# magnate3/dpdk_dc_sand

Measured on AMD Instinct MI355X. Metric: int8 voltage Gsamples/s ingested + beams/s, 64-ant 4096-ch; % HBM roofline, higher is better.
Workload: dtype int8

## Files before the change

### dpdk_dc_sand_amd/csrc/bf_fused.hpp

```cpp
#pragma once

#include <type_traits>

#include "bf_fused_plan.hpp"
#include "bf_mfma.hpp"
#include "bf_phase.hpp"

namespace bf {

typedef uint32_t u32x4_t __attribute__((ext_vector_type(4)));
typedef uint32_t u32x2_t __attribute__((ext_vector_type(2)));

struct FusedArgs {
  const uint8_t* raw;
  const float4* dv;
  const float* gain;
  const uint32_t* table;
  size_t table_bytes;
  void* y;
  int delay_channels, B, C, T, A, M, S, NT, nslabs, xcd_order;
  int path, order;
  int c_count;
  long long base_ch;
  double ctot, ts, k, t0, batch_dt;
  float out_scale;
  int ch_run;
};

__device__ __forceinline__ void apply_gain(float g, float* re, float* im) {
  *re = __fmul_rn(*re, g);
  *im = __fmul_rn(*im, g);
}


constexpr uint32_t kSelP0 = 0x05040100u;
constexpr uint32_t kSelP1 = 0x07060302u;
typedef int i32x4_t __attribute__((ext_vector_type(4)));

__device__ __forceinline__ i32x4_t mfma_i8(i32x4_t a, i32x4_t b, i32x4_t c) {
  return __builtin_amdgcn_mfma_i32_16x16x64_i8(a, b, c, 0, 0, 0);
}

__device__ __forceinline__ int coef8_byte(int k, int cl, int nts, int limb) {
  const int s = k >> 6, h = (k >> 4) & 3, j = k & 15, tau = cl >> 4, row = cl & 15;
  return ((((s * nts + tau) * 2 + limb) * 64) + row + 16 * h) * 16 + j;
}

template <bool Pow2 = false>
__device__ __forceinline__ uint32_t requant_bits(int y, float s) {
  constexpr float kMagic = 12582912.0f;
  float v;
  if constexpr (Pow2) {
    v = __builtin_fmaf(static_cast<float>(y), s, kMagic);
  } else {
#pragma clang fp contract(off)
    v = static_cast<float>(y) * s + kMagic;
  }
  return __float_as_uint(__builtin_amdgcn_fmed3f(v, kMagic - 127.0f, kMagic + 127.0f));
}

__device__ __forceinline__ uint32_t pack_low_bytes(uint32_t a, uint32_t b, uint32_t c, uint32_t d) {
  const uint32_t ab = __builtin_amdgcn_perm(b, a, 0x0c0c0400u);
  const uint32_t cd = __builtin_amdgcn_perm(d, c, 0x0c0c0400u);
  return __builtin_amdgcn_perm(cd, ab, 0x05040100u);
}

__device__ __forceinline__ void transpose_rows4(uint32_t (&v)[4]) {
  auto a = __builtin_amdgcn_permlane32_swap(v[0], v[2], false, false);
  auto b = __builtin_amdgcn_permlane32_swap(v[1], v[3], false, false);
  auto c = __builtin_amdgcn_permlane16_swap(a[0], b[0], false, false);
  auto d = __builtin_amdgcn_permlane16_swap(a[1], b[1], false, false);
  v[0] = c[0];
  v[1] = c[1];
  v[2] = d[0];
  v[3] = d[1];
}

__device__ __forceinline__ void lds_barrier() {
  __atomic_signal_fence(__ATOMIC_SEQ_CST);
  __builtin_amdgcn_s_waitcnt(0xc07f);
  __builtin_amdgcn_s_barrier();
  __atomic_signal_fence(__ATOMIC_SEQ_CST);
}

constexpr int kLayoutNatural = 0, kLayoutW32 = 1, kLayoutW32H = 2;
int launch_q14_table(const FusedArgs& P, uint32_t* out, int layout, hipStream_t st);

using FusedKernel = void (*)(FusedArgs);

template <class F>
FusedKernel with_bools(F f) {
  return f();
}
template <class F, class... Bs>
FusedKernel with_bools(F f, bool b, Bs... bs) {
  return b ? with_bools([&](auto... cs) -> FusedKernel { return f(std::true_type{}, cs...); }, bs...)
           : with_bools([&](auto... cs) -> FusedKernel { return f(std::false_type{}, cs...); }, bs...);
}

int launch_planned(FusedKernel k, const FusedPlan& p, FusedArgs P, hipStream_t st);
int launch_wide(const FusedPlan& p, FusedArgs P, hipStream_t st);
int launch_w32(const FusedPlan& p, FusedArgs P, hipStream_t st);

}
```

### dpdk_dc_sand_amd/csrc/bf_fused_dims.hpp

```cpp
#pragma once

#include <cstddef>
#include <cstdint>
#include <cstring>

#ifdef __HIPCC__
#define BF_HD __host__ __device__
#else
#define BF_HD
#endif

namespace bf {

constexpr size_t kMaxLds = 160 * 1024;

inline size_t coef_lds_bytes(int S, int nts) { return static_cast<size_t>(S) * nts * 2 * 64 * 16; }

constexpr int kGroup = 4;

constexpr int kF32StageRow = 36;
constexpr size_t kF32StageBytes = 4 * 64 * kF32StageRow * 4;

constexpr int kWideGroup = 2;
BF_HD inline int wide_padded_steps(int A) {
  return 2 * kWideGroup * ((((A + 15) >> 4) + 2 * kWideGroup - 1) / (2 * kWideGroup));
}
constexpr int kWidePSteps = 16;

constexpr int kW32Beams = 32;
constexpr int kW32TChannels = 4;
constexpr int kW32RChannels = 8;
BF_HD inline int w32_table_steps(int A) { return 4 * ((((A + 31) >> 5) + 3) / 4); }
BF_HD inline bool w32_table_fits(int A) { return w32_table_steps(A) <= 8; }
inline size_t w32_table_bytes(int B, int C, int A, int M) {
  return static_cast<size_t>(B) * C * ((M + 31) / 32) * 1024 * w32_table_steps(A) * 4;
}
BF_HD inline size_t w32_lds_bytes(int A) {
  return static_cast<size_t>(w32_table_steps(A)) * 4 * 2 * 64 * 16 + 4 * 64 * 4;
}

inline bool scale_is_pow2(float s) {
  uint32_t u;
  memcpy(&u, &s, 4);
  const uint32_t e = (u >> 23) & 255;
  return (u & 0x7fffffu) == 0 && e > 0 && e < 255;
}

}
```

### dpdk_dc_sand_amd/csrc/bf_fused_plan.cpp

```cpp
#include "bf_fused_plan.hpp"

#include <algorithm>
#include <cstdarg>
#include <cstdio>

namespace bf {
namespace {

FusedPlan refuse(const char* fmt, ...) __attribute__((format(printf, 1, 2)));
FusedPlan refuse(const char* fmt, ...) {
  FusedPlan p{};
  p.status = BF_ERR_ARG;
  va_list ap;
  va_start(ap, fmt);
  vsnprintf(p.error, sizeof(p.error), fmt, ap);
  va_end(ap);
  return p;
}

FusedPlan with_grid(FusedPlan p, long long grid, const char* too_large = "grid too large") {
  if (grid >= (1LL << 31)) return refuse("bf_beamform_fused: %s", too_large);
  p.grid = static_cast<unsigned>(grid);
  return p;
}

struct Shape : FusedShape {
  explicit Shape(const FusedShape& s) : FusedShape(s) {}
  int path() const { return flags & BF_FUSED_PATH_MASK; }
  int order() const { return flags & BF_FUSED_ORDER_MASK; }
  int S() const { return (2 * A + 31) / 32; }
  int S8() const { return (2 * A + 63) / 64; }
  int NT() const { return (2 * M + 15) / 16; }
  long long items() const { return static_cast<long long>(B) * C; }
  bool small() const { return A <= 64 && T <= 256; }
  bool offsets31() const { return static_cast<unsigned long long>(A) * C * T * 4 < (1ull << 31); }
  bool lane_offsets32(int rows) const {
    return static_cast<size_t>(rows) * C * T * 4 + static_cast<size_t>(T) * 4 < (1ull << 32);
  }
  bool slab_xcd_order(int nslabs) const { return nslabs > 1 && order() != BF_FUSED_ORDER_CHANNEL; }
  long long slab_grid(long long columns, int nslabs, bool xcd) const {
    return xcd ? (columns + 7) / 8 * 8 * nslabs : columns * nslabs;
  }
  bool item_xcd_order() const {
    if (order() == BF_FUSED_ORDER_CHANNEL) return false;
    if (order() == BF_FUSED_ORDER_XCD) return (C & 7) == 0;
    return (C & 7) == 0 && M >= 8;
  }
  bool wide_fits() const {
    return A >= 16 && lane_offsets32(12) && coef_lds_bytes(wide_padded_steps(A), 1) <= kMaxLds;
  }
  bool wide_p2_fits() const {
    return A == 256 && T == 256 && M % 32 == 0 && delay_channels == 1 && !gains && offsets31();
  }
  bool i8_w32_fits() const { return A >= 32 && (T & 1) == 0 && lane_offsets32(24) && w32_lds_bytes(A) <= kMaxLds; }
  bool w32r_fits() const {
    return w32_table_steps(A) == 8 && A > 224 && T == 256 && M % kW32Beams == 0 && offsets31() &&
           static_cast<unsigned long long>(B) * 2 * C * T * 2 * M < (1ull << 31);
  }
};

void item_slabs(const Shape& s, FusedPlan& p) {
  p.nts = s.NT() >= 2 ? 2 : 1;
  p.full = p.nts == 2 ? (2 * s.M) % 32 == 0 : 2 * s.M == 16;
  p.nslabs = (s.NT() + p.nts - 1) / p.nts;
  p.xcd_order = s.item_xcd_order();
}

FusedPlan plan_item(const Shape& s, FusedPlan p) {
  p.family = FusedFamily::Item;
  item_slabs(s, p);
  p.staged = !p.i8out && s.M == 16;
  p.pow2 = p.i8out && scale_is_pow2(s.out_scale);
  p.lds = coef_lds_bytes(s.S(), p.nts) + (p.staged ? kF32StageBytes : 0);
  return with_grid(p, p.nslabs * s.items(), "too many (batch, channel) items");
}

FusedPlan plan_generic(const Shape& s, FusedPlan p) {
  p.family = FusedFamily::Generic;
  p.nts = s.NT() >= 2 && coef_lds_bytes(s.S(), 2) <= kMaxLds ? 2 : 1;
  p.nslabs = (s.NT() + p.nts - 1) / p.nts;
  p.lds = coef_lds_bytes(s.S(), p.nts);
  if (p.lds > kMaxLds) return refuse("bf_beamform_fused: n_ants=%d too large", s.A);
  p.xcd_order = s.slab_xcd_order(p.nslabs);
  return with_grid(p, s.slab_grid(s.items(), p.nslabs, p.xcd_order));
}

FusedPlan plan_wide(const Shape& s, FusedPlan p) {
  if (!p.exact && s.wide_p2_fits() && s.order() != BF_FUSED_ORDER_CHANNEL) {
    p.family = FusedFamily::WideP2;
    p.nts = 2;
    p.nslabs = s.M / 32;
    const long long units = static_cast<long long>(s.B) * p.nslabs;
    const int cus = std::max(1, s.cus);
    p.ch_run = static_cast<int>(std::min<long long>(s.C, std::max<long long>(1, (s.C * units + cus - 1) / cus)));
    const long long groups = static_cast<long long>(s.B) * ((s.C + p.ch_run - 1) / p.ch_run);
    p.lds = 2 * coef_lds_bytes(kWidePSteps, 2);
    p.block = 512;
    return with_grid(p, s.slab_grid(groups, p.nslabs, true));
  }
  p.family = FusedFamily::Wide;
  const int Sp = wide_padded_steps(s.A);
  p.nts = s.M > 16 && coef_lds_bytes(Sp, 2) <= kMaxLds ? 2 : 1;
  p.buf = s.offsets31();
  p.lds = coef_lds_bytes(Sp, p.nts);
  p.nslabs = (s.M + 16 * p.nts - 1) / (16 * p.nts);
  p.xcd_order = s.slab_xcd_order(p.nslabs);
  return with_grid(p, s.slab_grid(s.items(), p.nslabs, p.xcd_order));
}

FusedPlan plan_i8_item(const Shape& s, FusedPlan p) {
  p.family = FusedFamily::I8Item;
  item_slabs(s, p);
  p.a64 = s.A == 64 && s.lane_offsets32(24);
  p.pow2 = scale_is_pow2(s.out_scale * 0x1p-14f);
  p.lds = static_cast<size_t>(2) * p.nts * 2 * 64 * 16 + 4 * 32 * 4;
  return with_grid(p, p.nslabs * s.items(), "too many items");
}

FusedPlan plan_i8_generic(const Shape& s, FusedPlan p) {
  p.family = FusedFamily::I8Generic;
  auto lds_bytes = [&](int nts) { return static_cast<size_t>(s.S8()) * nts * 2 * 64 * 16 + nts * 16 * 4; };
  p.nts = s.NT() >= 2 && lds_bytes(2) <= kMaxLds ? 2 : 1;
  p.lds = lds_bytes(p.nts);
  if (p.lds > kMaxLds) return refuse("bf_beamform_fused: n_ants=%d too large", s.A);
  p.nslabs = (s.NT() + p.nts - 1) / p.nts;
  return with_grid(p, s.items() * p.nslabs);
}

FusedPlan plan_w32(const Shape& s, FusedPlan p) {
  p.family = FusedFamily::W32;
  p.nslabs = (s.M + kW32Beams - 1) / kW32Beams;
  p.xcd_order = s.slab_xcd_order(p.nslabs);
  p.lds = w32_lds_bytes(s.A);
  p = with_grid(p, s.slab_grid(s.items(), p.nslabs, p.xcd_order));
  const size_t need = w32_table_bytes(s.B, s.C, s.A, s.M);
  if (p.status != BF_OK || !w32_table_fits(s.A) || s.workspace_bytes < need) return p;
  p.table = true;
  p.table_bytes = need;
  p.pow2 = scale_is_pow2(s.out_scale * 0x1p-14f);
  int channels;
  if (p.sgn && s.w32r_fits()) {
    p.family = FusedFamily::W32R;
    p.lds = 0;
    channels = kW32RChannels;
  } else {
    p.family = FusedFamily::W32T;
    const int npasses = ((((s.T >> 1) + 15) >> 4) + 3) >> 2;
    p.buf = s.offsets31();
    p.straight = w32_table_steps(s.A) == 8 && npasses == 2 && p.buf;
    p.pow2 = p.pow2 && p.straight;
    channels = p.straight ? 8 : kW32TChannels;
  }
  const long long groups = static_cast<long long>(s.B) * ((s.C + channels - 1) / channels);
  return with_grid(p, s.slab_grid(groups, p.nslabs, p.xcd_order));
}

}

FusedPlan plan_fused(const FusedShape& shape) {
  const Shape s(shape);
  FusedPlan p{};
  p.sgn = s.flags & BF_FUSED_SIGNED;
  p.i8out = s.flags & BF_FUSED_OUT_INT8;
  p.exact = s.flags & BF_FUSED_EXACT_COEFF;
  p.gain = s.gains;
  p.block = 256;
  const int path = s.path();
  const bool item = s.small() && path != BF_FUSED_PATH_GENERIC;
  if (p.i8out && !(s.flags & BF_FUSED_INT8_VIA_F32)) {
    if (!s.gains && static_cast<double>(s.A) * (p.sgn ? 128 : 255) * 23171.0 >= 2147483648.0)
      return refuse("bf_beamform_fused: n_ants=%d overflows the int8 path's int32 beam sums (%s samples); use float "
                    "beams or BF_FUSED_INT8_VIA_F32", s.A, p.sgn ? "int8" : "uint8");
    if ((path == BF_FUSED_PATH_WIDE || (path == 0 && !s.small())) && s.i8_w32_fits()) return plan_w32(s, p);
    return item ? plan_i8_item(s, p) : plan_i8_generic(s, p);
  }
  if (!p.i8out && (path == BF_FUSED_PATH_WIDE || (path == 0 && s.M >= 24 && (!s.small() || s.M > 32))) && s.wide_fits())
    return plan_wide(s, p);
  return item ? plan_item(s, p) : plan_generic(s, p);
}

const char* fused_family_name(FusedFamily f) {
  static const char* const names[] = {
      "beamform_fused_item_kernel",    "beamform_fused_kernel",        "beamform_fused_wide_kernel",
      "beamform_fused_wide_p2_kernel", "beamform_fused_i8_item_kernel", "beamform_fused_i8_kernel",
      "beamform_fused_i8_w32_kernel",  "beamform_fused_i8_w32t_kernel", "beamform_fused_i8_w32r_kernel"};
  return names[static_cast<int>(f)];
}

void fused_plan_name(const FusedPlan& p, char* out, size_t len) {
  const char* fam = fused_family_name(p.family);
  const char *io = p.i8out ? "i8" : "f32", *full = p.full ? "full" : "partial", *ex = p.exact ? "exact" : "fast";
  const char* scale = p.pow2 ? "pow2" : "anyscale";
  switch (p.family) {
    case FusedFamily::Item:
      snprintf(out, len, "%s:%s,nts%d,%s,%s%s%s%s", fam, io, p.nts, full, ex, p.staged ? ",staged" : "",
               p.i8out ? "," : "", p.i8out ? scale : "");
      break;
    case FusedFamily::Generic: snprintf(out, len, "%s:%s,nts%d,%s", fam, io, p.nts, ex); break;
    case FusedFamily::Wide:
      snprintf(out, len, "%s:tw%d,%s,%s,%s", fam, p.nts, ex, p.gain ? "gain" : "unit", p.buf ? "buf" : "ptr");
      break;
    case FusedFamily::WideP2: snprintf(out, len, "%s", fam); break;
    case FusedFamily::I8Item:
      snprintf(out, len, "%s:nts%d,%s,%s,%s", fam, p.nts, full, p.a64 ? "a64" : "aany", scale);
      break;
    case FusedFamily::I8Generic: snprintf(out, len, "%s:nts%d", fam, p.nts); break;
    case FusedFamily::W32: snprintf(out, len, "%s:%s", fam, p.gain ? "gain" : "unit"); break;
    case FusedFamily::W32T:
      if (p.straight) snprintf(out, len, "%s:straight,%s", fam, scale);
      else snprintf(out, len, "%s:general,%s", fam, p.buf ? "buf" : "ptr");
      break;
    case FusedFamily::W32R: snprintf(out, len, "%s:%s", fam, scale); break;
  }
}

}
```

### dpdk_dc_sand_amd/csrc/bf_fused_plan.hpp

```cpp
#pragma once

#include "../../include/bf.h"
#include "bf_fused_dims.hpp"

namespace bf {

enum class FusedFamily {
  Item,
  Generic,
  Wide,
  WideP2,
  I8Item,
  I8Generic,
  W32,
  W32T,
  W32R,
};

struct FusedShape {
  int B, C, T, A, M, delay_channels;
  bool gains;
  int flags;
  float out_scale;
  size_t workspace_bytes;
  int cus;
};

struct FusedPlan {
  int status;
  char error[200];
  FusedFamily family;
  bool sgn, i8out, exact;
  int nts;
  bool full, staged;
  bool a64, pow2;
  bool buf, gain;
  bool straight;
  bool table;
  size_t table_bytes;
  int nslabs, xcd_order, ch_run;
  size_t lds;
  unsigned grid, block;
};

FusedPlan plan_fused(const FusedShape& s);

const char* fused_family_name(FusedFamily f);
void fused_plan_name(const FusedPlan& p, char* out, size_t len);

}
```

### dpdk_dc_sand_amd/csrc/bf_wide_i8.hip

```cpp
#include <algorithm>
#include <cstdlib>
#include <type_traits>

#include "bf_fused.hpp"

namespace bf {

namespace {

constexpr int kW8Threads = 256;

__device__ __forceinline__ int w8_step_base(int s, int A) { return min(32 * s, A - 32); }
__host__ __device__ inline int w8_padded_steps(int A) { return 2 * ((((A + 31) >> 5) + 1) / 2); }


__host__ __device__ inline int w32_steps(int A) { return w32_table_steps(A); }

typedef uint16_t u16x2_t __attribute__((ext_vector_type(2)));

__device__ __forceinline__ void w32_expand_unit(int8_t* lb, int ml, int g, const u32x4_t& q0, const u32x4_t& q1) {
  const uint32_t d[8] = {q0[0], q0[1], q0[2], q0[3], q1[0], q1[1], q1[2], q1[3]};
  uint32_t n[8], np[8], pp[8];
#pragma unroll
  for (int i = 0; i < 8; ++i) {
    const u16x2_t v = __builtin_bit_cast(u16x2_t, d[i]);
    const u16x2_t neg = v * u16x2_t{1, 0xffff};
    n[i] = __builtin_bit_cast(uint32_t, neg);
    np[i] = __builtin_bit_cast(uint32_t, neg + u16x2_t{128, 128});
    pp[i] = __builtin_bit_cast(uint32_t, v + u16x2_t{128, 128});
  }
  u32x4_t e_hi0, e_lo0, e_hi1, e_lo1;
#pragma unroll
  for (int q = 0; q < 4; ++q) {
    e_lo0[q] = __builtin_amdgcn_perm(n[2 * q + 1], n[2 * q], 0x06040200u);
    e_hi0[q] = __builtin_amdgcn_perm(np[2 * q + 1], np[2 * q], 0x07050301u);
    e_lo1[q] = __builtin_amdgcn_perm(d[2 * q + 1], d[2 * q], 0x04060002u);
    e_hi1[q] = __builtin_amdgcn_perm(pp[2 * q + 1], pp[2 * q], 0x05070103u);
  }
  const int st = g >> 2, h = g & 3, tau = ml >> 3, row = (2 * ml) & 15;
  int8_t* o = lb + ((((st * 4 + tau) * 2) * 64) + row + 16 * h) * 16;
  *reinterpret_cast<u32x4_t*>(o) = e_hi0;
  *reinterpret_cast<u32x4_t*>(o + 64 * 16) = e_lo0;
  *reinterpret_cast<u32x4_t*>(o + 16) = e_hi1;
  *reinterpret_cast<u32x4_t*>(o + 16 + 64 * 16) = e_lo1;
}

__device__ __forceinline__ void w32_load(const uint8_t* __restrict__ base, size_t ant_stride, uint32_t loff, int s,
                                         int A, u32x2_t (&d)[8]) {
  const int a0 = w8_step_base(s, A);
#pragma unroll
  for (int q = 0; q < 8; ++q)
    d[q] = *reinterpret_cast<const u32x2_t*>(base + static_cast<size_t>(a0 + q) * ant_stride + loff);
}

__device__ __forceinline__ void w32_load_buf(__amdgpu_buffer_rsrc_t rs, uint32_t voff, uint32_t sbase, uint32_t stride,
                                             u32x2_t (&d)[8]) {
#pragma unroll
  for (int q = 0; q < 8; ++q)
    d[q] = __builtin_bit_cast(u32x2_t, __builtin_amdgcn_raw_buffer_load_b64(rs, voff, sbase + q * stride, 0));
}

template <bool Signed>
__device__ __forceinline__ void w32_frags(const u32x2_t (&d)[8], i32x4_t (&f)[2][2]) {
#pragma unroll
  for (int p = 0; p < 2; ++p)
#pragma unroll
    for (int i = 0; i < 2; ++i) {
      uint32_t w[4];
#pragma unroll
      for (int m2 = 0; m2 < 4; ++m2) {
        const u32x2_t da = d[2 * m2], db = d[2 * m2 + 1];
        uint32_t a = i ? da.y : da.x, b = i ? db.y : db.x;
        if constexpr (!Signed) {
          a ^= 0x80808080u;
          b ^= 0x80808080u;
        }
        w[m2] = __builtin_amdgcn_perm(b, a, p ? kSelP1 : kSelP0);
      }
      f[p][i] = i32x4_t{static_cast<int>(w[0]), static_cast<int>(w[1]), static_cast<int>(w[2]), static_cast<int>(w[3])};
    }
}

__device__ __forceinline__ void w32_mfma(const int4* __restrict__ fr, int s, int lane, const i32x4_t (&f)[2][2],
                                         i32x4_t (&hi)[2][2][4], i32x4_t (&lo)[2][2][4]) {
#pragma unroll
  for (int t = 0; t < 4; ++t) {
    const int4 x0 = fr[(((s * 4 + t) * 2 + 0) * 64) + lane];
    const int4 x1 = fr[(((s * 4 + t) * 2 + 1) * 64) + lane];
    const i32x4_t chi = i32x4_t{x0.x, x0.y, x0.z, x0.w}, clo = i32x4_t{x1.x, x1.y, x1.z, x1.w};
#pragma unroll
    for (int p = 0; p < 2; ++p)
#pragma unroll
      for (int i = 0; i < 2; ++i) {
        hi[p][i][t] = mfma_i8(chi, f[p][i], hi[p][i][t]);
        lo[p][i][t] = mfma_i8(clo, f[p][i], lo[p][i][t]);
      }
  }
}

template <bool Signed, bool Gain = false>
__global__ __launch_bounds__(kW8Threads, 2) void beamform_fused_i8_w32_kernel(FusedArgs P) {
  extern __shared__ __attribute__((aligned(16))) int4 lds4[];
  const int tid = threadIdx.x, lane = tid & 63, wave = tid >> 6;
  const int h = lane >> 4, tl = lane & 15;
  int slab, bc;
  if (P.xcd_order) {
    const int x = blockIdx.x & 7, local = blockIdx.x >> 3;
    slab = local % P.nslabs;
    bc = (local / P.nslabs) * 8 + x;
    if (bc >= P.B * P.C) return;
  } else {
    slab = blockIdx.x % P.nslabs;
    bc = blockIdx.x / P.nslabs;
  }
  const int b = bc / P.C, c = bc % P.C;
  const int m0 = slab * kW32Beams;
  const int Sp = w32_steps(P.A);
  const int T2 = P.T >> 1;
  const int nchunks = (T2 + 15) >> 4;
  const int npasses = (nchunks + 3) >> 2;
  const size_t ant_stride = static_cast<size_t>(P.C) * P.T * 4;
  const uint32_t hoff = static_cast<uint32_t>(8 * h) * static_cast<uint32_t>(ant_stride);
  const uint8_t* base = P.raw + (static_cast<size_t>(b) * P.A * P.C + c) * static_cast<size_t>(P.T) * 4;
  int8_t* lb = reinterpret_cast<int8_t*>(lds4);
  int* partial = reinterpret_cast<int*>(lb + static_cast<size_t>(Sp) * 4 * 2 * 64 * 16);

  __builtin_assume(Sp >= 4 && (Sp & 3) == 0 && npasses >= 1);
  const int total = npasses * Sp;
  int issued = 0, ls = 0, lchunk = wave;
  auto issue = [&](u32x2_t (&d)[8]) {
    const uint32_t loff = hoff + static_cast<uint32_t>(min(lchunk * 16 + tl, T2 - 1)) * 8u;
    w32_load(base, ant_stride, loff, ls, P.A, d);
    ++issued;
    const bool adv = issued < total;
    const bool wrap = ls + 1 == Sp;
    ls = adv ? (wrap ? 0 : ls + 1) : ls;
    lchunk = (adv && wrap) ? lchunk + 4 : lchunk;
  };
  const int ml = (tid >> 2) & (kW32Beams - 1);
  const int sa0 = 4 * (tid >> 7) + (tid & 3);
  const bool m_ok = m0 + ml < P.M;
  const float4* dv_row =
      P.dv + (static_cast<size_t>(P.delay_channels == 1 ? 0 : c) * P.M + min(m0 + ml, P.M - 1)) * P.A;
  const float* g_row = Gain ? P.gain + static_cast<size_t>(min(m0 + ml, P.M - 1)) * P.A : nullptr;
  constexpr int kBatch = 8;
  auto batch_model = [&](int j0, float4 (&dv)[kBatch], float (&gv)[kBatch]) {
#pragma unroll
    for (int j = 0; j < kBatch; ++j) {
      const int sa = sa0 + 8 * (j0 + j), st = sa >> 5;
      const int a = min(w8_step_base(st, P.A) + (sa & 31), P.A - 1);
      dv[j] = dv_row[a];
      if constexpr (Gain)
        gv[j] = g_row[a];
      else
        gv[j] = 1.0f;
    }
  };
  float4 dv_first[kBatch];
  float gv_first[kBatch];
  batch_model(0, dv_first, gv_first);
  __builtin_amdgcn_sched_barrier(0);

  u32x2_t d0[8], d1[8], d2[8], d3[8];
  issue(d0);
  issue(d1);
  issue(d2);
  issue(d3);
  __builtin_amdgcn_sched_barrier(0);

  {
    const double dt = P.t0 + static_cast<double>(b) * P.batch_dt;
// ... 217 lines not shown
      const int ml = tid & 31;
      int cs0 = 0, cs1 = 0;
#pragma unroll
      for (int j = 0; j < 4; ++j) {
        if (2 * j >= Sp) break;
        w32_expand_unit(lb, ml, (tid >> 5) + 8 * j, tq[j][0], tq[j][1]);
        if constexpr (!Signed) {
#pragma unroll
          for (int hf = 0; hf < 2; ++hf)
#pragma unroll
            for (int q = 0; q < 4; ++q) {
              const int wc = static_cast<int16_t>(tq[j][hf][q] & 0xffffu), ws = static_cast<int>(tq[j][hf][q]) >> 16;
              cs0 += wc - ws;
              cs1 += ws + wc;
            }
        }
      }
      if constexpr (!Signed) {
        cs0 += __shfl_xor(cs0, 32);
        cs1 += __shfl_xor(cs1, 32);
        if (lane < 32) {
          partial[wave * 64 + 2 * ml] = cs0;
          partial[wave * 64 + 2 * ml + 1] = cs1;
        }
      }
    }
    lds_barrier();
    if constexpr (!Signed) {
      if (tid < 64) partial[tid] += partial[64 + tid] + partial[128 + tid] + partial[192 + tid];
      lds_barrier();
    }
    auto run_pass = [&](int pass, auto last) {
      constexpr bool kLast = decltype(last)::value;
      const int tq2 = (wave + 4 * pass) * 16 + tl;
      i32x4_t hi[2][2][4], lo[2][2][4];
#pragma unroll
      for (int p = 0; p < 2; ++p)
#pragma unroll
        for (int i = 0; i < 2; ++i)
#pragma unroll
          for (int t = 0; t < 4; ++t) hi[p][i][t] = lo[p][i][t] = i32x4_t{0, 0, 0, 0};
      if constexpr (kSp != 0) {
#pragma unroll
        for (int s = 0; s < kSp; ++s) {
          i32x4_t f[2][2];
          const int j = (pass * kSp + s) % NB;
          w32_frags<Signed>(db[j], f);
          __builtin_amdgcn_sched_barrier(0);
          issue(db[j]);
          w32_mfma(lds4, s, lane, f, hi, lo);
          __builtin_amdgcn_sched_barrier(0);
        }
      } else {
        for (int s = 0; s < Sp; s += 2) {
          i32x4_t f[2][2];
#pragma unroll
          for (int j = 0; j < 2; ++j) {
            w32_frags<Signed>(db[j], f);
            issue(db[j]);
            w32_mfma(lds4, s + j, lane, f, hi, lo);
          }
        }
      }
      constexpr bool next_table = kLast && Early;
#pragma unroll
      for (int p = 0; p < 2; ++p) {
        if constexpr (next_table)
          if (p == 1) {
            __builtin_amdgcn_sched_barrier(0);
            load_table(min(kc + 1, nk - 1));
            __builtin_amdgcn_sched_barrier(0);
          }
        uint32_t pk[2][4];
#pragma unroll
        for (int i = 0; i < 2; ++i)
#pragma unroll
          for (int t = 0; t < 4; ++t) {
            uint32_t qb[4];
            int4 cs = int4{0, 0, 0, 0};
            if constexpr (!Signed) cs = reinterpret_cast<const int4*>(partial)[4 * t + h];
            const int csr[4] = {cs.x, cs.y, cs.z, cs.w};
#pragma unroll
            for (int r = 0; r < 4; ++r) {
              int y = (hi[p][i][t][r] << 8) + lo[p][i][t][r];
              if constexpr (!Signed) y += 128 * csr[r];
              qb[r] = requant_bits<Pow2>(y, s32);
            }
            pk[i][t] = pack_low_bytes(qb[0], qb[1], qb[2], qb[3]);
          }
        const size_t prow = ((static_cast<size_t>(b) * 2 + p) * P.C + c) * static_cast<size_t>(P.T);
        if (full) {
#pragma unroll
          for (int i = 0; i < 2; ++i) transpose_rows4(pk[i]);
          if (tq2 < T2) {
#pragma unroll
            for (int i = 0; i < 2; ++i) {
              int8_t* o = reinterpret_cast<int8_t*>(P.y) + (prow + 2 * tq2 + i) * M2 + 2 * m0 + 16 * h;
              *reinterpret_cast<u32x4_t*>(o) = u32x4_t{pk[i][0], pk[i][1], pk[i][2], pk[i][3]};
            }
          }
        } else if (tq2 < T2) {
#pragma unroll
          for (int i = 0; i < 2; ++i) {
            int8_t* o = reinterpret_cast<int8_t*>(P.y) + (prow + 2 * tq2 + i) * M2 + 2 * m0;
#pragma unroll
            for (int t = 0; t < 4; ++t)
#pragma unroll
              for (int r = 0; r < 4; ++r) {
                const int col = 16 * t + 4 * h + r;
                if (2 * m0 + col < M2) o[col] = static_cast<int8_t>((pk[i][t] >> (8 * r)) & 255);
              }
          }
        }
      }
    };
    if constexpr (Early) {
      if constexpr (kNP != 0) {
#pragma unroll
        for (int pass = 0; pass + 1 < kNP; ++pass) run_pass(pass, std::false_type{});
      } else {
        for (int pass = 0; pass + 1 < npasses; ++pass) run_pass(pass, std::false_type{});
      }
      run_pass(npasses - 1, std::true_type{});
    } else {
      if constexpr (kNP != 0) {
#pragma unroll
        for (int pass = 0; pass < kNP; ++pass) run_pass(pass, std::false_type{});
      } else {
        for (int pass = 0; pass < npasses; ++pass) run_pass(pass, std::false_type{});
      }
      load_table(min(kc + 1, nk - 1));
    }
    if constexpr (kSp != 0 && (kSp * kNP) % NB != 0) {
      constexpr int r = (kSp * kNP) % NB;
      u32x2_t tmp[NB][8];
#pragma unroll
      for (int j = 0; j < NB; ++j)
#pragma unroll
        for (int q = 0; q < 8; ++q) tmp[j][q] = db[(j + r) % NB][q];
#pragma unroll
      for (int j = 0; j < NB; ++j)
#pragma unroll
        for (int q = 0; q < 8; ++q) db[j][q] = tmp[j][q];
    }
    if (kc + 1 < nk) lds_barrier();
  }
}

__shared__ __attribute__((aligned(16))) int4 w32r_img[8 * 2 * 2 * 64];
__shared__ __attribute__((aligned(16))) int4 w32r_slot0[4 * 256];
__shared__ __attribute__((aligned(16))) int4 w32r_slot1[4 * 256];
__shared__ __attribute__((aligned(16))) int w32r_ws[4 * 32];

typedef __attribute__((address_space(3))) void* lds_void_ptr;

__device__ __forceinline__ void w32r_expand_unit(int4* img, int ml, int g, const u32x4_t& q0, const u32x4_t& q1) {
  const uint32_t d[8] = {q0[0], q0[1], q0[2], q0[3], q1[0], q1[1], q1[2], q1[3]};
  uint32_t n[8], np[8];
#pragma unroll
  for (int i = 0; i < 8; ++i) {
    const u16x2_t neg = __builtin_bit_cast(u16x2_t, d[i]) * u16x2_t{1, 0xffff};
    n[i] = __builtin_bit_cast(uint32_t, neg);
    np[i] = __builtin_bit_cast(uint32_t, neg + u16x2_t{128, 128});
  }
  u32x4_t ehi, elo;
#pragma unroll
  for (int q = 0; q < 4; ++q) {
    elo[q] = __builtin_amdgcn_perm(n[2 * q + 1], n[2 * q], 0x06040200u);
    ehi[q] = __builtin_amdgcn_perm(np[2 * q + 1], np[2 * q], 0x07050301u);
  }
  int4* o = img + ((g >> 2) * 2 + (ml >> 4)) * 2 * 64 + (ml & 15) + 16 * (g & 3);
  o[0] = __builtin_bit_cast(int4, ehi);
  o[64] = __builtin_bit_cast(int4, elo);
}

__device__ __forceinline__ i32x4_t w32r_frag_im(const i32x4_t& f) {
  i32x4_t r;
#pragma unroll
  for (int q = 0; q < 4; ++q) {
    const uint32_t n = static_cast<uint32_t>(f[q]) ^ 0x00ff00ffu;
    r[q] = static_cast<int>(__builtin_amdgcn_perm(n, n, 0x02030001u));
  }
  return r;
}

template <bool Pow2>
__global__ __launch_bounds__(kW8Threads, 2) void beamform_fused_i8_w32r_kernel(FusedArgs P) {
  constexpr int Sp = 8, NP = 2, kCh = kW32RChannels;
  const int tid = threadIdx.x, lane = tid & 63;
  const int wave = __builtin_amdgcn_readfirstlane(tid >> 6);
  const int h = lane >> 4, tl = lane & 15;
  const int C = P.C;
  const int gpb = (C + kCh - 1) / kCh;
  int slab, grp;
  if (P.xcd_order) {
    const int x = blockIdx.x & 7, local = blockIdx.x >> 3;
    slab = local % P.nslabs;
    grp = (local / P.nslabs) * 8 + x;
    if (grp >= P.B * gpb) return;
  } else {
    slab = blockIdx.x % P.nslabs;
    grp = blockIdx.x / P.nslabs;
  }
  const int b = grp / gpb, c0 = (grp - b * gpb) * kCh;
  const int nk = min(kCh, C - c0);
  const int m0 = slab * kW32Beams;
  const uint32_t ant_stride = static_cast<uint32_t>(C) * static_cast<uint32_t>(P.T) * 4u;
  const uint32_t ch_bytes = static_cast<uint32_t>(P.T) * 4u;
  const uint8_t* base = P.raw + (static_cast<size_t>(b) * P.A * C + c0) * static_cast<size_t>(P.T) * 4;
  const __amdgpu_buffer_rsrc_t vrs = __builtin_amdgcn_make_buffer_rsrc(const_cast<uint8_t*>(base), 0, 0x7fffffff,
                                                                        0x00020000);
  const uint32_t dma_voff = static_cast<uint32_t>(8 * ((lane >> 3) & 3) + (lane >> 5)) * ant_stride +
                            16u * static_cast<uint32_t>(lane & 7);
  int4* const slot0 = w32r_slot0 + 256 * wave;
  int4* const slot1 = w32r_slot1 + 256 * wave;

  const int total = nk * NP * Sp;
  int issued = 0, ls = 0, lp = 0, lk = 0;
  auto dma_sb = [&]() {
    return __builtin_amdgcn_readfirstlane(static_cast<uint32_t>(w8_step_base(ls, P.A)) * ant_stride +
                                          static_cast<uint32_t>(lk) * ch_bytes +
                                          static_cast<uint32_t>(wave + 4 * lp) * 128u);
  };
  auto dma_piece = [&](int4* slot, int k, uint32_t sb) {
    __builtin_amdgcn_raw_ptr_buffer_load_lds(vrs, (lds_void_ptr)(slot + 64 * k), 16, dma_voff,
                                             sb + 2u * static_cast<uint32_t>(k) * ant_stride, 0, 0);
  };
  auto advance = [&]() {
    ++issued;
    const bool adv = issued < total;
    const bool wrap = ls + 1 == Sp, pwrap = lp + 1 == NP;
    ls = adv ? (wrap ? 0 : ls + 1) : ls;
    lp = (adv && wrap) ? (pwrap ? 0 : lp + 1) : lp;
    lk = (adv && wrap && pwrap) ? lk + 1 : lk;
  };
  auto dma = [&](int4* slot) {
    const uint32_t sb = dma_sb();
#pragma unroll
    for (int k = 0; k < 4; ++k) dma_piece(slot, k, sb);
    advance();
  };
  auto read_slot = [&](const int4* slot, u32x2_t (&d)[8]) {
    const u32x2_t* s2 = reinterpret_cast<const u32x2_t*>(slot);
#pragma unroll
    for (int q = 0; q < 8; ++q) d[q] = s2[(4 * q + h) * 16 + tl];
  };

  const u32x4_t* tbase = reinterpret_cast<const u32x4_t*>(P.table) +
                         ((static_cast<size_t>(b) * C + c0) * P.nslabs + slab) * 256 * Sp;
  const size_t tstride = static_cast<size_t>(P.nslabs) * 256 * Sp;
  u32x4_t tq[4][2];
  auto load_table = [&](int kc) {
    const __amdgpu_buffer_rsrc_t rs = __builtin_amdgcn_make_buffer_rsrc(
        const_cast<u32x4_t*>(tbase + static_cast<size_t>(kc) * tstride), 0, 0x7fffffff, 0x00020000);
#pragma unroll
    for (int j = 0; j < 4; ++j)
#pragma unroll
      for (int hf = 0; hf < 2; ++hf)
        tq[j][hf] = __builtin_bit_cast(
            u32x4_t, __builtin_amdgcn_raw_buffer_load_b128(rs, static_cast<uint32_t>(((j * 2 + hf) * 256 + tid) * 16), 0, 0));
  };
  auto expand = [&]() {
    const int ml = tid & 31;
    int ws = 0;
#pragma unroll
    for (int j = 0; j < 4; ++j) {
      w32r_expand_unit(w32r_img, ml, (tid >> 5) + 8 * j, tq[j][0], tq[j][1]);
#pragma unroll
      for (int hf = 0; hf < 2; ++hf)
#pragma unroll
        for (int q = 0; q < 4; ++q) ws += static_cast<int>(tq[j][hf][q]) >> 16;
    }
    ws += __shfl_xor(ws, 32);
    if (lane < 32) w32r_ws[32 * wave + ml] = ws;
  };

  load_table(0);
  __builtin_amdgcn_sched_barrier(0);
  dma(slot0);
  dma(slot1);
  __builtin_amdgcn_sched_barrier(0);
  expand();
  lds_barrier();

  const float s32 = P.out_scale * 0x1p-14f;
  const int M2 = 2 * P.M;
  const __amdgpu_buffer_rsrc_t yrs = __builtin_amdgcn_make_buffer_rsrc(P.y, 0, 0x7fffffff, 0x00020000);
  const uint32_t so_lane = static_cast<uint32_t>(2 * tl * M2 + 16 * (h >> 1) + 32 * (h & 1));
  for (int kc = 0; kc < nk; ++kc) {
    const int c = c0 + kc;
#pragma unroll
    for (int pass = 0; pass < NP; ++pass) {
      i32x4_t rh[2][2][2], rl[2][2][2], ih[2][2][2], il[2][2][2];
#pragma unroll
      for (int p = 0; p < 2; ++p)
#pragma unroll
        for (int i = 0; i < 2; ++i)
#pragma unroll
          for (int t = 0; t < 2; ++t) rh[p][i][t] = rl[p][i][t] = ih[p][i][t] = il[p][i][t] = i32x4_t{0, 0, 0, 0};
#pragma unroll
      for (int s = 0; s < Sp; ++s) {
        int4* const slot = (s & 1) ? slot1 : slot0;
        u32x2_t d[8];
        read_slot(slot, d);
        i32x4_t f[2][2], fi[2][2];
        w32_frags<true>(d, f);
#pragma unroll
        for (int p = 0; p < 2; ++p)
#pragma unroll
          for (int i = 0; i < 2; ++i) fi[p][i] = w32r_frag_im(f[p][i]);
        asm volatile("" ::"v"(f[0][0]), "v"(f[0][1]), "v"(f[1][0]), "v"(f[1][1]) : "memory");
        __builtin_amdgcn_sched_barrier(0);
        const uint32_t sb = dma_sb();
#pragma unroll
        for (int t = 0; t < 2; ++t) {
          const int4 x0 = w32r_img[((s * 2 + t) * 2 + 0) * 64 + lane];
          const int4 x1 = w32r_img[((s * 2 + t) * 2 + 1) * 64 + lane];
          const i32x4_t ahi = i32x4_t{x0.x, x0.y, x0.z, x0.w}, alo = i32x4_t{x1.x, x1.y, x1.z, x1.w};
#pragma unroll
          for (int p = 0; p < 2; ++p) {
            __builtin_amdgcn_sched_barrier(0);
            dma_piece(slot, 2 * t + p, sb);
            __builtin_amdgcn_sched_barrier(0);
#pragma unroll
            for (int i = 0; i < 2; ++i) {
              rh[p][i][t] = mfma_i8(ahi, f[p][i], rh[p][i][t]);
              rl[p][i][t] = mfma_i8(alo, f[p][i], rl[p][i][t]);
              ih[p][i][t] = mfma_i8(ahi, fi[p][i], ih[p][i][t]);
              il[p][i][t] = mfma_i8(alo, fi[p][i], il[p][i][t]);
            }
          }
        }
        advance();
        __builtin_amdgcn_sched_barrier(0);
      }
      if (pass == NP - 1) {
        __builtin_amdgcn_sched_barrier(0);
        load_table(min(kc + 1, nk - 1));
        __builtin_amdgcn_sched_barrier(0);
      }
      int bias[2][4];
#pragma unroll
      for (int t = 0; t < 2; ++t) {
        int4 acc = int4{0, 0, 0, 0};
#pragma unroll
        for (int w = 0; w < 4; ++w) {
          const int4 v = *reinterpret_cast<const int4*>(w32r_ws + 32 * w + 16 * t + 4 * h);
          acc.x += v.x;
          acc.y += v.y;
          acc.z += v.z;
          acc.w += v.w;
        }
        bias[t][0] = -acc.x;
        bias[t][1] = -acc.y;
        bias[t][2] = -acc.z;
        bias[t][3] = -acc.w;
      }
#pragma unroll
      for (int p = 0; p < 2; ++p) {
        const uint32_t prow = static_cast<uint32_t>(((b * 2 + p) * C + c) * P.T);
#pragma unroll
        for (int i = 0; i < 2; ++i) {
          uint32_t pk[2][2];
#pragma unroll
          for (int t = 0; t < 2; ++t) {
            uint32_t qr[4], qi[4];
#pragma unroll
            for (int r = 0; r < 4; ++r) {
              qr[r] = requant_bits<Pow2>((rh[p][i][t][r] << 8) + rl[p][i][t][r], s32);
              qi[r] = requant_bits<Pow2>((ih[p][i][t][r] << 8) + il[p][i][t][r] + bias[t][r], s32);
            }
            pk[t][0] = pack_low_bytes(qr[0], qi[0], qr[1], qi[1]);
            pk[t][1] = pack_low_bytes(qr[2], qi[2], qr[3], qi[3]);
          }
          const auto sw0 = __builtin_amdgcn_permlane16_swap(pk[0][0], pk[1][0], false, false);
          const auto sw1 = __builtin_amdgcn_permlane16_swap(pk[0][1], pk[1][1], false, false);
          const u32x4_t sd = u32x4_t{sw0[0], sw1[0], sw0[1], sw1[1]};
          const uint32_t soff = (prow + static_cast<uint32_t>(2 * (wave + 4 * pass) * 16 + i)) * static_cast<uint32_t>(M2) +
                                static_cast<uint32_t>(2 * m0);
          __builtin_amdgcn_raw_buffer_store_b128(sd, yrs, so_lane, soff, 0);
          __builtin_amdgcn_sched_barrier(0);
          asm volatile("s_nop 1");
          __builtin_amdgcn_sched_barrier(0);
        }
      }
    }
    if (kc + 1 < nk) {
      lds_barrier();
      expand();
      lds_barrier();
    }
  }
  asm volatile("s_waitcnt vmcnt(0)" ::: "memory");
}

template <bool Signed>
FusedKernel w32_kernel(const FusedPlan& p) {
  if constexpr (Signed)
    if (p.family == FusedFamily::W32R)
      return with_bools([](auto pow2) -> FusedKernel { return beamform_fused_i8_w32r_kernel<pow2.value>; }, p.pow2);
  if (p.family == FusedFamily::W32T) {
    if (p.straight)
      return with_bools([](auto pow2) -> FusedKernel {
        return beamform_fused_i8_w32t_kernel<Signed, false, 8, 2, 2, 8, true, pow2.value>;
      }, p.pow2);
    return with_bools([](auto buf) -> FusedKernel {
      return beamform_fused_i8_w32t_kernel<Signed, false, 0, 0, 4, kW32TChannels, buf.value, false>;
    }, p.buf);
  }
  return with_bools([](auto gain) -> FusedKernel { return beamform_fused_i8_w32_kernel<Signed, gain.value>; }, p.gain);
}

}

int launch_w32(const FusedPlan& p, FusedArgs P, hipStream_t st) {
  if (p.table) {
    const int e = launch_q14_table(P, const_cast<uint32_t*>(P.table), kLayoutW32, st);
    if (e != BF_OK) return e;
  }
  return launch_planned(!p.sgn ? w32_kernel<false>(p) : w32_kernel<true>(p), p, P, st);
}

}
```

Measured before the change: 2478.

## Add 64-beam-wide W32R int8 beamform kernel with CU-sized channel runs

```diff
diff --git a/dpdk_dc_sand_amd/csrc/bf_fused.hpp b/dpdk_dc_sand_amd/csrc/bf_fused.hpp
--- a/dpdk_dc_sand_amd/csrc/bf_fused.hpp
+++ b/dpdk_dc_sand_amd/csrc/bf_fused.hpp
@@ -101,5 +101,6 @@
 int launch_planned(FusedKernel k, const FusedPlan& p, FusedArgs P, hipStream_t st);
 int launch_wide(const FusedPlan& p, FusedArgs P, hipStream_t st);
 int launch_w32(const FusedPlan& p, FusedArgs P, hipStream_t st);
+FusedKernel w32r_b64_kernel(const FusedPlan& p);
 
 }
diff --git a/dpdk_dc_sand_amd/csrc/bf_fused_dims.hpp b/dpdk_dc_sand_amd/csrc/bf_fused_dims.hpp
--- a/dpdk_dc_sand_amd/csrc/bf_fused_dims.hpp
+++ b/dpdk_dc_sand_amd/csrc/bf_fused_dims.hpp
@@ -30,6 +30,7 @@
 constexpr int kW32Beams = 32;
 constexpr int kW32TChannels = 4;
 constexpr int kW32RChannels = 8;
+constexpr int kW32RWideBeams = 64;
 BF_HD inline int w32_table_steps(int A) { return 4 * ((((A + 31) >> 5) + 3) / 4); }
 BF_HD inline bool w32_table_fits(int A) { return w32_table_steps(A) <= 8; }
 inline size_t w32_table_bytes(int B, int C, int A, int M) {
diff --git a/dpdk_dc_sand_amd/csrc/bf_fused_plan.cpp b/dpdk_dc_sand_amd/csrc/bf_fused_plan.cpp
--- a/dpdk_dc_sand_amd/csrc/bf_fused_plan.cpp
+++ b/dpdk_dc_sand_amd/csrc/bf_fused_plan.cpp
@@ -139,10 +139,20 @@
   p.table_bytes = need;
   p.pow2 = scale_is_pow2(s.out_scale * 0x1p-14f);
   int channels;
+  int columns = p.nslabs;
   if (p.sgn && s.w32r_fits()) {
     p.family = FusedFamily::W32R;
     p.lds = 0;
     channels = kW32RChannels;
+    p.b64 = s.M % kW32RWideBeams == 0 && s.order() != BF_FUSED_ORDER_CHANNEL;
+    if (p.b64) {
+      p.block = 512;
+      columns = s.M / kW32RWideBeams;
+      const long long units = static_cast<long long>(s.B) * s.C * columns;
+      const int cus = std::max(1, s.cus);
+      channels = static_cast<int>(std::min<long long>(s.C, std::max<long long>(channels, (units + cus - 1) / cus)));
+      p.ch_run = channels;
+    }
   } else {
     p.family = FusedFamily::W32T;
     const int npasses = ((((s.T >> 1) + 15) >> 4) + 3) >> 2;
@@ -152,7 +162,7 @@
     channels = p.straight ? 8 : kW32TChannels;
   }
   const long long groups = static_cast<long long>(s.B) * ((s.C + channels - 1) / channels);
-  return with_grid(p, s.slab_grid(groups, p.nslabs, p.xcd_order));
+  return with_grid(p, s.slab_grid(groups, columns, p.xcd_order));
 }
 
 }
diff --git a/dpdk_dc_sand_amd/csrc/bf_fused_plan.hpp b/dpdk_dc_sand_amd/csrc/bf_fused_plan.hpp
--- a/dpdk_dc_sand_amd/csrc/bf_fused_plan.hpp
+++ b/dpdk_dc_sand_amd/csrc/bf_fused_plan.hpp
@@ -36,6 +36,7 @@
   bool a64, pow2;
   bool buf, gain;
   bool straight;
+  bool b64;
   bool table;
   size_t table_bytes;
   int nslabs, xcd_order, ch_run;
diff --git a/dpdk_dc_sand_amd/csrc/bf_wide_i8.hip b/dpdk_dc_sand_amd/csrc/bf_wide_i8.hip
--- a/dpdk_dc_sand_amd/csrc/bf_wide_i8.hip
+++ b/dpdk_dc_sand_amd/csrc/bf_wide_i8.hip
@@ -3,6 +3,7 @@
 #include <type_traits>
 
 #include "bf_fused.hpp"
+#include "bf_wide_i8.hpp"
 
 namespace bf {
 
@@ -10,13 +11,10 @@
 
 constexpr int kW8Threads = 256;
 
-__device__ __forceinline__ int w8_step_base(int s, int A) { return min(32 * s, A - 32); }
 __host__ __device__ inline int w8_padded_steps(int A) { return 2 * ((((A + 31) >> 5) + 1) / 2); }
 
 
 __host__ __device__ inline int w32_steps(int A) { return w32_table_steps(A); }
-
-typedef uint16_t u16x2_t __attribute__((ext_vector_type(2)));
 
 __device__ __forceinline__ void w32_expand_unit(int8_t* lb, int ml, int g, const u32x4_t& q0, const u32x4_t& q1) {
   const uint32_t d[8] = {q0[0], q0[1], q0[2], q0[3], q1[0], q1[1], q1[2], q1[3]};
@@ -540,37 +538,6 @@
 __shared__ __attribute__((aligned(16))) int4 w32r_slot1[4 * 256];
 __shared__ __attribute__((aligned(16))) int w32r_ws[4 * 32];
 
-typedef __attribute__((address_space(3))) void* lds_void_ptr;
-
-__device__ __forceinline__ void w32r_expand_unit(int4* img, int ml, int g, const u32x4_t& q0, const u32x4_t& q1) {
-  const uint32_t d[8] = {q0[0], q0[1], q0[2], q0[3], q1[0], q1[1], q1[2], q1[3]};
-  uint32_t n[8], np[8];
-#pragma unroll
-  for (int i = 0; i < 8; ++i) {
-    const u16x2_t neg = __builtin_bit_cast(u16x2_t, d[i]) * u16x2_t{1, 0xffff};
-    n[i] = __builtin_bit_cast(uint32_t, neg);
-    np[i] = __builtin_bit_cast(uint32_t, neg + u16x2_t{128, 128});
-  }
-  u32x4_t ehi, elo;
-#pragma unroll
-  for (int q = 0; q < 4; ++q) {
-    elo[q] = __builtin_amdgcn_perm(n[2 * q + 1], n[2 * q], 0x06040200u);
-    ehi[q] = __builtin_amdgcn_perm(np[2 * q + 1], np[2 * q], 0x07050301u);
-  }
-  int4* o = img + ((g >> 2) * 2 + (ml >> 4)) * 2 * 64 + (ml & 15) + 16 * (g & 3);
-  o[0] = __builtin_bit_cast(int4, ehi);
-  o[64] = __builtin_bit_cast(int4, elo);
-}
-
-__device__ __forceinline__ i32x4_t w32r_frag_im(const i32x4_t& f) {
-  i32x4_t r;
-#pragma unroll
-  for (int q = 0; q < 4; ++q) {
-    const uint32_t n = static_cast<uint32_t>(f[q]) ^ 0x00ff00ffu;
-    r[q] = static_cast<int>(__builtin_amdgcn_perm(n, n, 0x02030001u));
-  }
-  return r;
-}
 
 template <bool Pow2>
 __global__ __launch_bounds__(kW8Threads, 2) void beamform_fused_i8_w32r_kernel(FusedArgs P) {
@@ -806,6 +773,7 @@
     const int e = launch_q14_table(P, const_cast<uint32_t*>(P.table), kLayoutW32, st);
     if (e != BF_OK) return e;
   }
+  if (p.family == FusedFamily::W32R && p.b64) return launch_planned(w32r_b64_kernel(p), p, P, st);
   return launch_planned(!p.sgn ? w32_kernel<false>(p) : w32_kernel<true>(p), p, P, st);
 }
 
diff --git a/dpdk_dc_sand_amd/csrc/bf_wide_i8.hpp b/dpdk_dc_sand_amd/csrc/bf_wide_i8.hpp
--- /dev/null
+++ b/dpdk_dc_sand_amd/csrc/bf_wide_i8.hpp
@@ -0,0 +1,44 @@
+#pragma once
+
+#include "bf_fused.hpp"
+
+namespace bf {
+
+__device__ __forceinline__ int w8_step_base(int s, int A) { return min(32 * s, A - 32); }
+
+typedef uint16_t u16x2_t __attribute__((ext_vector_type(2)));
+
+typedef __attribute__((address_space(3))) void* lds_void_ptr;
+
+template <int kTiles = 2>
+__device__ __forceinline__ void w32r_expand_unit(int4* img, int ml, int g, const u32x4_t& q0, const u32x4_t& q1) {
+  const uint32_t d[8] = {q0[0], q0[1], q0[2], q0[3], q1[0], q1[1], q1[2], q1[3]};
+  uint32_t n[8], np[8];
+#pragma unroll
+  for (int i = 0; i < 8; ++i) {
+    const u16x2_t neg = __builtin_bit_cast(u16x2_t, d[i]) * u16x2_t{1, 0xffff};
+    n[i] = __builtin_bit_cast(uint32_t, neg);
+    np[i] = __builtin_bit_cast(uint32_t, neg + u16x2_t{128, 128});
+  }
+  u32x4_t ehi, elo;
+#pragma unroll
+  for (int q = 0; q < 4; ++q) {
+    elo[q] = __builtin_amdgcn_perm(n[2 * q + 1], n[2 * q], 0x06040200u);
+    ehi[q] = __builtin_amdgcn_perm(np[2 * q + 1], np[2 * q], 0x07050301u);
+  }
+  int4* o = img + ((g >> 2) * kTiles + (ml >> 4)) * 2 * 64 + (ml & 15) + 16 * (g & 3);
+  o[0] = __builtin_bit_cast(int4, ehi);
+  o[64] = __builtin_bit_cast(int4, elo);
+}
+
+__device__ __forceinline__ i32x4_t w32r_frag_im(const i32x4_t& f) {
+  i32x4_t r;
+#pragma unroll
+  for (int q = 0; q < 4; ++q) {
+    const uint32_t n = static_cast<uint32_t>(f[q]) ^ 0x00ff00ffu;
+    r[q] = static_cast<int>(__builtin_amdgcn_perm(n, n, 0x02030001u));
+  }
+  return r;
+}
+
+}
diff --git a/dpdk_dc_sand_amd/csrc/bf_wide_i8_b64.hip b/dpdk_dc_sand_amd/csrc/bf_wide_i8_b64.hip
--- /dev/null
+++ b/dpdk_dc_sand_amd/csrc/bf_wide_i8_b64.hip
@@ -0,0 +1,241 @@
+#include "bf_fused.hpp"
+#include "bf_wide_i8.hpp"
+
+namespace bf {
+
+namespace b64 {
+
+constexpr int kThreads = 512, kWaves = 8;
+
+__shared__ __attribute__((aligned(16))) int4 img[8 * 4 * 2 * 64];
+__shared__ __attribute__((aligned(16))) int4 slot0[kWaves * 128];
+__shared__ __attribute__((aligned(16))) int4 slot1[kWaves * 128];
+__shared__ __attribute__((aligned(16))) int ws_part[4 * 64];
+
+__device__ __forceinline__ void frags(const uint32_t (&d)[8], i32x4_t (&f)[2]) {
+#pragma unroll
+  for (int p = 0; p < 2; ++p) {
+    uint32_t w[4];
+#pragma unroll
+    for (int m2 = 0; m2 < 4; ++m2) w[m2] = __builtin_amdgcn_perm(d[2 * m2 + 1], d[2 * m2], p ? kSelP1 : kSelP0);
+    f[p] = i32x4_t{static_cast<int>(w[0]), static_cast<int>(w[1]), static_cast<int>(w[2]), static_cast<int>(w[3])};
+  }
+}
+
+template <bool Pow2>
+__global__ __launch_bounds__(kThreads, 1) void beamform_fused_i8_w32r_kernel(FusedArgs P) {
+  constexpr int Sp = 8, NP = 2;
+  const int kCh = P.ch_run;
+  const int tid = threadIdx.x, lane = tid & 63;
+  const int wave = __builtin_amdgcn_readfirstlane(tid >> 6);
+  const int h = lane >> 4, tl = lane & 15;
+  const int C = P.C;
+  const int gpb = (C + kCh - 1) / kCh;
+  const int ncols = P.nslabs >> 1;
+  int col, grp;
+  if (P.xcd_order) {
+    const int x = blockIdx.x & 7, local = blockIdx.x >> 3;
+    col = local % ncols;
+    grp = (local / ncols) * 8 + x;
+    if (grp >= P.B * gpb) return;
+  } else {
+    col = blockIdx.x % ncols;
+    grp = blockIdx.x / ncols;
+  }
+  const int b = grp / gpb, c0 = (grp - b * gpb) * kCh;
+  const int nk = min(kCh, C - c0);
+  const uint32_t ant_stride = static_cast<uint32_t>(C) * static_cast<uint32_t>(P.T) * 4u;
+  const uint32_t ch_bytes = static_cast<uint32_t>(P.T) * 4u;
+  const uint8_t* base = P.raw + (static_cast<size_t>(b) * P.A * C + c0) * static_cast<size_t>(P.T) * 4;
+  const __amdgpu_buffer_rsrc_t vrs = __builtin_amdgcn_make_buffer_rsrc(const_cast<uint8_t*>(base), 0, 0x7fffffff,
+                                                                        0x00020000);
+  const uint32_t dma_voff = static_cast<uint32_t>(8 * ((lane >> 2) & 3) + (lane >> 4)) * ant_stride +
+                            16u * static_cast<uint32_t>(lane & 3);
+  int4* const s0 = slot0 + 128 * wave;
+  int4* const s1 = slot1 + 128 * wave;
+
+  const int total = nk * NP * Sp;
+  int issued = 0, ls = 0, lp = 0, lk = 0;
+  auto dma_sb = [&]() {
+    return __builtin_amdgcn_readfirstlane(static_cast<uint32_t>(w8_step_base(ls, P.A)) * ant_stride +
+                                          static_cast<uint32_t>(lk) * ch_bytes +
+                                          static_cast<uint32_t>(wave + kWaves * lp) * 64u);
+  };
+  auto dma_piece = [&](int4* slot, int k, uint32_t sb) {
+    __builtin_amdgcn_raw_ptr_buffer_load_lds(vrs, (lds_void_ptr)(slot + 64 * k), 16, dma_voff,
+                                             sb + 4u * static_cast<uint32_t>(k) * ant_stride, 0, 0);
+  };
+  auto advance = [&]() {
+    ++issued;
+    const bool adv = issued < total;
+    const bool wrap = ls + 1 == Sp, pwrap = lp + 1 == NP;
+    ls = adv ? (wrap ? 0 : ls + 1) : ls;
+    lp = (adv && wrap) ? (pwrap ? 0 : lp + 1) : lp;
+    lk = (adv && wrap && pwrap) ? lk + 1 : lk;
+  };
+  auto dma = [&](int4* slot) {
+    const uint32_t sb = dma_sb();
+#pragma unroll
+    for (int k = 0; k < 2; ++k) dma_piece(slot, k, sb);
+    advance();
+  };
+  auto read_slot = [&](const int4* slot, uint32_t (&d)[8]) {
+    const uint32_t* s4 = reinterpret_cast<const uint32_t*>(slot);
+#pragma unroll
+    for (int q = 0; q < 8; ++q) d[q] = s4[(4 * q + h) * 16 + tl];
+  };
+
+  const int half = tid >> 8, t8 = tid & 255;
+  const u32x4_t* tbase = reinterpret_cast<const u32x4_t*>(P.table) +
+                         ((static_cast<size_t>(b) * C + c0) * P.nslabs + 2 * col) * 256 * Sp;
+  const size_t tstride = static_cast<size_t>(P.nslabs) * 256 * Sp;
+  u32x4_t tq[4][2];
+  constexpr int kNonTemporal = 2;
+  auto load_table = [&](int kc) {
+    const __amdgpu_buffer_rsrc_t rs = __builtin_amdgcn_make_buffer_rsrc(
+        const_cast<u32x4_t*>(tbase + static_cast<size_t>(kc) * tstride), 0, 0x7fffffff, 0x00020000);
+#pragma unroll
+    for (int j = 0; j < 4; ++j)
+#pragma unroll
+      for (int hf = 0; hf < 2; ++hf)
+        tq[j][hf] = __builtin_bit_cast(
+            u32x4_t, __builtin_amdgcn_raw_buffer_load_b128(
+                         rs, static_cast<uint32_t>(((half * Sp + j * 2 + hf) * 256 + t8) * 16), 0, kNonTemporal));
+  };
+  auto expand = [&]() {
+    const int ml = 32 * half + (t8 & 31);
+    int ws = 0;
+#pragma unroll
+    for (int j = 0; j < 4; ++j) {
+      w32r_expand_unit<4>(img, ml, (t8 >> 5) + 8 * j, tq[j][0], tq[j][1]);
+#pragma unroll
+      for (int hf = 0; hf < 2; ++hf)
+#pragma unroll
+        for (int q = 0; q < 4; ++q) ws += static_cast<int>(tq[j][hf][q]) >> 16;
+    }
+    ws += __shfl_xor(ws, 32);
+    if (lane < 32) ws_part[64 * (wave & 3) + ml] = ws;
+  };
+
+  load_table(0);
+  __builtin_amdgcn_sched_barrier(0);
+  dma(s0);
+  dma(s1);
+  __builtin_amdgcn_sched_barrier(0);
+  expand();
+  lds_barrier();
+
+  const float s32 = P.out_scale * 0x1p-14f;
+  const int M2 = 2 * P.M;
+  const __amdgpu_buffer_rsrc_t yrs = __builtin_amdgcn_make_buffer_rsrc(P.y, 0, 0x7fffffff, 0x00020000);
+  const uint32_t so_lane = static_cast<uint32_t>(tl * M2 + 16 * (h >> 1) + 32 * (h & 1));
+  for (int kc = 0; kc < nk; ++kc) {
+    const int c = c0 + kc;
+#pragma unroll
+    for (int pass = 0; pass < NP; ++pass) {
+      i32x4_t rh[2][4], rl[2][4], ih[2][4], il[2][4];
+#pragma unroll
+      for (int p = 0; p < 2; ++p)
+#pragma unroll
+        for (int t = 0; t < 4; ++t) rh[p][t] = rl[p][t] = ih[p][t] = il[p][t] = i32x4_t{0, 0, 0, 0};
+#pragma unroll
+      for (int s = 0; s < Sp; ++s) {
+        int4* const slot = (s & 1) ? s1 : s0;
+        uint32_t d[8];
+        read_slot(slot, d);
+        i32x4_t f[2], fi[2];
+        frags(d, f);
+#pragma unroll
+        for (int p = 0; p < 2; ++p) fi[p] = w32r_frag_im(f[p]);
+        asm volatile("" ::"v"(f[0]), "v"(f[1]) : "memory");
+        __builtin_amdgcn_sched_barrier(0);
+        const uint32_t sb = dma_sb();
+#pragma unroll
+        for (int t = 0; t < 4; ++t) {
+          const int4 x0 = img[((s * 4 + t) * 2 + 0) * 64 + lane];
+          const int4 x1 = img[((s * 4 + t) * 2 + 1) * 64 + lane];
+          const i32x4_t ahi = i32x4_t{x0.x, x0.y, x0.z, x0.w}, alo = i32x4_t{x1.x, x1.y, x1.z, x1.w};
+          if ((t & 1) == 0) {
+            __builtin_amdgcn_sched_barrier(0);
+            dma_piece(slot, t >> 1, sb);
+            __builtin_amdgcn_sched_barrier(0);
+          }
+#pragma unroll
+          for (int p = 0; p < 2; ++p) {
+            rh[p][t] = mfma_i8(ahi, f[p], rh[p][t]);
+            rl[p][t] = mfma_i8(alo, f[p], rl[p][t]);
+            ih[p][t] = mfma_i8(ahi, fi[p], ih[p][t]);
+            il[p][t] = mfma_i8(alo, fi[p], il[p][t]);
+          }
+        }
+        advance();
+        __builtin_amdgcn_sched_barrier(0);
+      }
+      if (pass == NP - 1) {
+        __builtin_amdgcn_sched_barrier(0);
+        load_table(min(kc + 1, nk - 1));
+        __builtin_amdgcn_sched_barrier(0);
+      }
+      int bias[4][4];
+#pragma unroll
+      for (int t = 0; t < 4; ++t) {
+        int4 acc = int4{0, 0, 0, 0};
+#pragma unroll
+        for (int w = 0; w < 4; ++w) {
+          const int4 v = *reinterpret_cast<const int4*>(ws_part + 64 * w + 16 * t + 4 * h);
+          acc.x += v.x;
+          acc.y += v.y;
+          acc.z += v.z;
+          acc.w += v.w;
+        }
+        bias[t][0] = -acc.x;
+        bias[t][1] = -acc.y;
+        bias[t][2] = -acc.z;
+        bias[t][3] = -acc.w;
+      }
+#pragma unroll
+      for (int p = 0; p < 2; ++p) {
+        const uint32_t prow = static_cast<uint32_t>(((b * 2 + p) * C + c) * P.T);
+#pragma unroll
+        for (int u = 0; u < 2; ++u) {
+          uint32_t pk[2][2];
+#pragma unroll
+          for (int j = 0; j < 2; ++j) {
+            const int t = 2 * u + j;
+            uint32_t qr[4], qi[4];
+#pragma unroll
+            for (int r = 0; r < 4; ++r) {
+              qr[r] = requant_bits<Pow2>((rh[p][t][r] << 8) + rl[p][t][r], s32);
+              qi[r] = requant_bits<Pow2>((ih[p][t][r] << 8) + il[p][t][r] + bias[t][r], s32);
+            }
+            pk[j][0] = pack_low_bytes(qr[0], qi[0], qr[1], qi[1]);
+            pk[j][1] = pack_low_bytes(qr[2], qi[2], qr[3], qi[3]);
+          }
+          const auto sw0 = __builtin_amdgcn_permlane16_swap(pk[0][0], pk[1][0], false, false);
+          const auto sw1 = __builtin_amdgcn_permlane16_swap(pk[0][1], pk[1][1], false, false);
+          const u32x4_t sd = u32x4_t{sw0[0], sw1[0], sw0[1], sw1[1]};
+          const uint32_t soff = (prow + static_cast<uint32_t>((wave + kWaves * pass) * 16)) * static_cast<uint32_t>(M2) +
+                                static_cast<uint32_t>(2 * kW32RWideBeams * col + 64 * u);
+          __builtin_amdgcn_raw_buffer_store_b128(sd, yrs, so_lane, soff, 0);
+          __builtin_amdgcn_sched_barrier(0);
+          asm volatile("s_nop 1");
+          __builtin_amdgcn_sched_barrier(0);
+        }
+      }
+    }
+    if (kc + 1 < nk) {
+      lds_barrier();
+      expand();
+      lds_barrier();
+    }
+  }
+  asm volatile("s_waitcnt vmcnt(0)" ::: "memory");
+}
+
+}
+
+FusedKernel w32r_b64_kernel(const FusedPlan& p) {
+  return with_bools([](auto pow2) -> FusedKernel { return b64::beamform_fused_i8_w32r_kernel<pow2.value>; }, p.pow2);
+}
+
+}
```

Result: no change. 2470 (-0.3%).
